# BenjSta/bernoulli-var-speech-codec

Hardware: AMD Instinct MI355X
Metric: audio-seconds coded per wall-second (encode+decode), 22.05 kHz @ 3 kbit/s (higher is better)
Workload: dtype f32; 1 GPU; BASELINE configs[1]: batch 64 x 5 s utterances per GPU, config_varBitRate @ 3000 bit/s (35 bits/frame), full encode -> BigVGAN decode; one batch at a time on one stream; frames_per_utterance=430, weights=seeded synthetic (checkpoints are LFS pointers), gather=none, streams=1

## Files before the change

bernoulli-var-speech-codec_amd/_abi.py:

```python
import ctypes
import os

import torch

_HERE = os.path.dirname(os.path.abspath(__file__))
LIB_PATH = os.environ.get("BVC_LIB") or os.path.join(_HERE, "csrc", "libbvcodec_hip.so")

c_float_p = ctypes.POINTER(ctypes.c_float)


class BvcConfig(ctypes.Structure):
    _fields_ = [
        ("num_mels", ctypes.c_int32), ("h_dim", ctypes.c_int32), ("z_dim", ctypes.c_int32),
        ("var_bit", ctypes.c_int32), ("n_fft", ctypes.c_int32), ("hop", ctypes.c_int32),
        ("pad_left", ctypes.c_int32), ("sample_rate", ctypes.c_int32),
        ("fmin", ctypes.c_float), ("fmax", ctypes.c_float),
        ("upsample_initial_channel", ctypes.c_int32), ("n_up", ctypes.c_int32),
        ("up_rates", ctypes.c_int32 * 8), ("up_kernels", ctypes.c_int32 * 8),
        ("n_resk", ctypes.c_int32), ("res_kernels", ctypes.c_int32 * 4),
        ("res_dilations", (ctypes.c_int32 * 3) * 4),
    ]


class BvcTensor(ctypes.Structure):
# ... 22 lines not shown
                                         _vp, _sz, _vp]),
    "bvc_bigvgan": (ctypes.c_int, [_vp, _vp, _i32, _i64, _i64, _f, _vp, _vp, _sz, _vp]),
    "bvc_vocoder_stream_create": (ctypes.c_int, [_vp, _i32, _i32, ctypes.POINTER(_vp)]),
    "bvc_vocoder_stream_destroy": (None, [_vp]),
    "bvc_vocoder_stream_reset": (ctypes.c_int, [_vp, _vp]),
    "bvc_vocoder_stream_push": (ctypes.c_int, [_vp, _vp, _i32, _f, _vp, _vp]),
    "bvc_stream_codec_create": (ctypes.c_int, [_vp, _i32, _i32, _f, _f, _f, ctypes.POINTER(_vp)]),
    "bvc_stream_codec_destroy": (None, [_vp]),
    "bvc_stream_codec_buffers": (ctypes.c_int, [_vp, ctypes.POINTER(_vp), ctypes.POINTER(_vp), ctypes.POINTER(_vp), ctypes.POINTER(_i32)]),
    "bvc_stream_codec_tick": (ctypes.c_int, [_vp, ctypes.POINTER(_i32), _vp]),
    "bvc_stream_codec_open": (ctypes.c_int, [_vp, _i32, _f, ctypes.POINTER(_i32)]),
    "bvc_stream_codec_close": (ctypes.c_int, [_vp, _i32]),
    "bvc_stream_codec_set_bits": (ctypes.c_int, [_vp, _i32, _f]),
    "bvc_stream_codec_slot_frames": (ctypes.c_int, [_vp, _i32, ctypes.POINTER(_i32), ctypes.POINTER(_i32), ctypes.POINTER(_i64)]),
    "bvc_encode": (ctypes.c_int, [_vp, _vp, _i32, _i64, _f, _f, _vp, _vp, _sz, _vp]),
    "bvc_decode": (ctypes.c_int, [_vp, _vp, _i32, _i64, _i64, _f, _vp, _vp, _sz, _vp]),
    "bvc_forward": (ctypes.c_int, [_vp, _vp, _i32, _i64, _f, _f, _i64, _f, _vp, _vp, _vp, _sz, _vp]),
    "bvc_encode_ragged": (ctypes.c_int, [_vp, _vp, _vp, _i32, _i64, _f, _vp, _f, _vp, _vp, _sz, _vp]),
    "bvc_decode_ragged": (ctypes.c_int, [_vp, _vp, _vp, _i32, _i64, _vp, _i64, _f, _vp, _vp, _sz, _vp]),
    "bvc_resample_poly": (ctypes.c_int, [_vp, _i32, _i64, _vp, _i32, _i32, _i32, _i64, _vp, _i64, _vp]),
    "bvc_peak_normalize": (ctypes.c_int, [_vp, _i32, _i64, _vp]),
    "bvc_pack_codes": (ctypes.c_int, [_vp, _i32, _i64, _i32, _i32, _vp, _vp]),
    "bvc_unpack_codes": (ctypes.c_int, [_vp, _i32, _i64, _i32, _i32, _vp, _vp]),
    "bvc_probe_begin": (ctypes.c_int, [_i32, _i32, _i32]),
    "bvc_probe_end": (ctypes.c_int, [ctypes.POINTER(ctypes.c_double), ctypes.POINTER(ctypes.c_double),
                                     ctypes.POINTER(_i32)]),
    "bvc_kprobe_enable": (ctypes.c_int, [_i32]),
    "bvc_kprobe_read": (ctypes.c_int, [_i32, _i32, ctypes.POINTER(ctypes.c_double), ctypes.POINTER(ctypes.c_double),
                                       ctypes.POINTER(_i32)]),
    "bvc_kprobe_read_span": (ctypes.c_int, [_i32, _i32, _i32, _i32, ctypes.POINTER(ctypes.c_double),
                                            ctypes.POINTER(ctypes.c_double), ctypes.POINTER(_i32)]),
    "bvc_test_linear": (ctypes.c_int, [_vp, _vp, _vp, _i32, _i32, _i32, _i32, _vp, _vp]),
    "bvc_test_linear_batched": (ctypes.c_int, [_vp, _vp, _vp, _i32, _i32, _i32, _i32, _vp, _vp]),
    "bvc_test_snakebeta": (ctypes.c_int, [_vp, _i64, _f, _f, _vp, _vp]),
    "bvc_test_vocoder_tap": (ctypes.c_int, [_vp, _vp, _i32, _i64, _i32, _vp, ctypes.POINTER(_i64), _vp, _sz, _vp]),
}

_lib = None


class BvcError(RuntimeError):
    pass


def load():
    global _lib
    if _lib is None:
        if not os.path.exists(LIB_PATH):
            raise BvcError(f"{LIB_PATH} is missing: build it with `python -m bvcodec.build` "
                           "(or __graft_entry__.build()); this package has no CPU fallback")
        lib = ctypes.CDLL(LIB_PATH)
        for name, (res, args) in SIGNATURES.items():
            fn = getattr(lib, name)
            fn.restype, fn.argtypes = res, args
        if lib.bvc_abi_version() != 3:
            raise BvcError("libbvcodec_hip.so ABI version mismatch")
        _lib = lib
    return _lib


def check(rc):
    if rc != 0:
        msg = load().bvc_last_error()
        raise BvcError(f"bvcodec error {rc}: {msg.decode() if msg else ''}")


# ... 10 lines not shown
```

bernoulli-var-speech-codec_amd/csrc/bvc_internal.h:

```cpp
#pragma once
#include <hip/hip_runtime.h>
#include <stdint.h>
#include <string>
#include <vector>

#include "../../include/bvcodec.h"

namespace bvc {

void set_error(const char *fmt, ...);

#define BVC_HIP_TRY(expr)                                                              \
    do {                                                                               \
        hipError_t e_ = (expr);                                                        \
        if (e_ != hipSuccess) {                                                        \
            bvc::set_error("%s failed: %s (%s:%d)", #expr, hipGetErrorString(e_), __FILE__, __LINE__); \
            return BVC_EHIP;                                                           \
        }                                                                              \
    } while (0)

enum ProbeKind { PK_NONE = 0, PK_LINEAR = 1, PK_GRU = 2, PK_CONV = 3, PK_BATCHED = 4, PK_STFT = 5, PK_POST = 6 };
struct ProbeScope {
    hipStream_t s; int slot;
    ProbeScope(int kind, hipStream_t stream);
// ... 48 lines not shown
};
enum CodeSample {
    CS_ENCODE = 0,
    CS_GREEDY = 1,
    CS_SAMPLE = 2
};

struct GemmParams {
    int     M, N;
    int     nb_total;
    int     gate_rows;
    GemmSeg seg[3];
    int     nseg;
    int     var_bit;
    int     sample;
    int     gate_il;
    const float *bias0;
    const float *bias1;
    DynPtr  y, y2, y3;
    DynPtr  aux;
    const float *part_i; const float *part_h; long long ldpart;
    const float *mean; const float *stdv;
    const CallDesc *desc;
    unsigned long long *probe;
    int     node;
    int     tstep;
    int     frames;
};

int launch_gemm_skinny(const GemmParams &p, int epi, hipStream_t s, int mtw = 1);
int skinny_kernels_init();
int launch_step_advance(CallDesc *d, int by, hipStream_t s);
int launch_set_desc(CallDesc *d, const CallDesc &v, hipStream_t s);

enum GemmOut { GO_NATURAL = 0, GO_FRAME_MAJOR_ROWS = 1, GO_PACKED_FRAMES = 2, GO_PACKED_FROM_UTT = 3 };
int launch_gemm_batched(const float *x, long long ldx, const float *w, long long ldw, const float *bias,
                        int M, int N, int K, int act, float *y, long long ldy, hipStream_t s,
                        int out_mode = GO_NATURAL, long long frames_T = 0, int mt16 = 0);
int launch_normalize_rows(const float *y, const float *mean, const float *stdv, long long rows, int n,
                          float *out, hipStream_t s);
int launch_fill(float *p, float v, long long n, hipStream_t s);
int launch_kld_frames(const float *prob, const float *prior, const float *bits, int B, long long T, int Z, float *kld,
                      hipStream_t s);
int launch_copy_rows(const float *src, long long lds, float *dst, long long ldd, int rows, int n, hipStream_t s);
int launch_repack_rows(const float *src, float *dst, long long ld_natural, int rows, int n, int dir, hipStream_t s);

constexpr unsigned FLOW_POISON = 0xFFFFDEADu;
constexpr int FLOW_STAMPS = 6;
enum FlowEpi { FE_ELU = 0, FE_CODE = 1, FE_MEL = 2, FE_GRU = 3, FE_ELU_KEEP = 4 };
enum FlowBuf { FB_H = 0, FB_E1, FB_E2, FB_ZC, FB_Q1, FB_Q2, FB_Q3, FB_D1, FB_D2, FB_D3, FB_DN, FB_G1, FB_G2, FB_G3, FB_COUNT };
struct FlowLin {
    const float *w;
    const float *bias;
    int wnb;
    int pad_;
};
struct FlowArgs {
    FlowLin enc0h, enc1, enc2, pz0, pz1, pz2, dec0h, dec0z, dec1, dec2, dec3, px0, px1, px2;
    const float *w_hh, *w_ihx, *w_ihz;
    const float *b_ih, *b_hh;
    int hb, zb, xb;
    float *flow; unsigned slot_bytes;
    int B, MT, NTG;
    long long T;
    const float *part0;
    const float *part_gru;
// ... 90 lines not shown
```

bernoulli-var-speech-codec_amd/csrc/bvcodec_abi.hip:

```cpp
#include <algorithm>
#include <atomic>
#include <cmath>
#include <cstdarg>
#include <cstdio>
#include <cstdlib>
#include <cstring>
#include <list>
#include <map>
#include <memory>
#include <mutex>

#include "bvc_internal.h"

namespace bvc {

static thread_local char g_err[512] = "";

void set_error(const char *fmt, ...) {
    va_list ap;
    va_start(ap, fmt);
    vsnprintf(g_err, sizeof(g_err), fmt, ap);
    va_end(ap);
}

// ... 2432 lines not shown
                }
                const unsigned long long b = h[(size_t)to * per + t * g_kprobe.nodes + k];
                if (!a || b <= a) continue;
                const double us = (double)(b - a) * 0.01;
                sum += us; if (us < mn) mn = us; ++n;
            }
    }
    if (mean_us) *mean_us = n ? sum / n : 0.0;
    if (min_us) *min_us = n ? mn : 0.0;
    if (n_samples) *n_samples = n;
    return BVC_OK;
}

int bvc_test_linear(const float *d_x, const float *d_w, const float *d_bias, int32_t M, int32_t N, int32_t K,
                    int32_t act, float *d_y, void *stream) {
    if (K % 16 || N % 16) { set_error("bvc_test_linear: N and K must be multiples of 16"); return BVC_EINVAL; }
    float *wp = nullptr;
    BVC_HIP_TRY(hipMalloc(reinterpret_cast<void **>(&wp), (size_t)N * K * sizeof(float)));
    hipStream_t s = (hipStream_t)stream;
    int rc = launch_repack_rows(d_w, wp, K, N, K, 0, s);
    Linear l; l.w = d_w; l.wp = wp; l.b = d_bias; l.in = K; l.out = N;
    if (!rc) rc = launch_gemm_skinny(lin_params(l, dp_static(d_x, K), M, dp_static(d_y, N)), act ? EPI_ELU : EPI_LINEAR, s);
    hipError_t e = hipStreamSynchronize(s);
    (void)hipFree(wp);
    if (!rc && e != hipSuccess) { set_error("bvc_test_linear: %s", hipGetErrorString(e)); rc = BVC_EHIP; }
    return rc;
}

int bvc_test_linear_batched(const float *d_x, const float *d_w, const float *d_bias, int32_t M, int32_t N, int32_t K,
                            int32_t act, float *d_y, void *stream) {
    return launch_gemm_batched(d_x, K, d_w, K, d_bias, M, N, K, act, d_y, N, (hipStream_t)stream);
}

int bvc_test_snakebeta(const float *d_x, int64_t n, float alpha, float beta, float *d_y, void *stream) {
    if (!d_x || !d_y || n <= 0) { set_error("bvc_test_snakebeta: bad arguments"); return BVC_EINVAL; }
    const float a = (float)std::exp((double)alpha);
    const float ib = 1.0f / ((float)std::exp((double)beta) + 0.000000001f);
    return launch_snakebeta_test(d_x, n, a, ib, d_y, (hipStream_t)stream);
}

int bvc_test_vocoder_tap(const bvc_model *m, const float *d_mel, int32_t B, int64_t T, int32_t which, float *d_out,
                         int64_t *out_numel_per_batch, void *d_ws, size_t ws_bytes, void *stream) {
    Workspace w;
    int rc = check_ws(m, B, T, d_ws, ws_bytes, &w);
    if (rc) return rc;
    if (which < 0 || which > 2 * m->cfg.n_up) { set_error("tap index out of range"); return BVC_EINVAL; }
    const float *tap = nullptr;
    int64_t len = 0;
    int ch = 0;
    hipStream_t s = (hipStream_t)stream;
    if ((rc = run_vocoder(m, w, d_mel, B, T, 1, 1.0f, nullptr, which, &tap, &len, &ch, s))) return rc;
    const long long n = (long long)B * len * ch;
    if (out_numel_per_batch) *out_numel_per_batch = len * ch;
    if (d_out) {
        hipLaunchKernelGGL(tap_copy_kernel, dim3(1024), dim3(256), 0, s, tap, d_out, n);
        BVC_HIP_TRY(hipGetLastError());
    }
    return BVC_OK;
}

}
```

bernoulli-var-speech-codec_amd/csrc/k_gemm.hip:

```cpp
#include <cstdlib>

#include <cstdint>
#include <type_traits>

#include "bvc_internal.h"

namespace bvc {

typedef float f32x4 __attribute__((ext_vector_type(4)));

__device__ __forceinline__ f32x4 mfma16(float a, float b, f32x4 c) {
    return __builtin_amdgcn_mfma_f32_16x16x4f32(a, b, c, 0, 0, 0);
}

__device__ __forceinline__ float elu1(float v) { return v > 0.0f ? v : expf(v) - 1.0f; }
__device__ __forceinline__ float sigmoid1(float v) { return 1.0f / (1.0f + expf(-v)); }

struct Resolved { float *p; long long ld; bool ok; int packed; };

__device__ __forceinline__ int sload_i32(const void *p) {
    int v;
    asm volatile("s_load_dword %0, %1, 0x0\n\ts_waitcnt lgkmcnt(0)" : "=s"(v) : "s"(p) : "memory");
    return v;
}
__device__ __forceinline__ long long sload_i64(const void *p) {
    long long v;
    asm volatile("s_load_dwordx2 %0, %1, 0x0\n\ts_waitcnt lgkmcnt(0)" : "=s"(v) : "s"(p) : "memory");
    return v;
}

template <bool MF = false>
__device__ __forceinline__ Resolved resolve(const DynPtr &d, const CallDesc *c, int mt16, int tstep) {
// ... 590 lines not shown
            if (row >= M) continue;
#pragma unroll
            for (int j = 0; j < 4; ++j) {
                const int col = n0 + j * 16 + g * 4;
                const f32x4 b4 = bias ? *reinterpret_cast<const f32x4 *>(bias + col) : (f32x4){0.f, 0.f, 0.f, 0.f};
                f32x4 v = acc[i][j] + b4;
                if (ACT == 1) {
#pragma unroll
                    for (int e = 0; e < 4; ++e) v[e] = elu1(v[e]);
                }
                *reinterpret_cast<f32x4 *>(y + out_index(row, col, N, ldy, frames_T, mt16, out_mode)) = v;
            }
        }
        return;
    }
#pragma unroll
    for (int j = 0; j < 4; ++j) {
        const int col = n0 + j * 16 + r;
        const float b = bias ? bias[col] : 0.0f;
#pragma unroll
        for (int i = 0; i < MI; ++i)
#pragma unroll
            for (int e = 0; e < 4; ++e) {
                const int row = m0 + i * 16 + g * 4 + e;
                if (row < M) {
                    float v = acc[i][j][e] + b;
                    if (ACT == 1) v = elu1(v);
                    y[out_index(row, col, N, ldy, frames_T, mt16, out_mode)] = v;
                }
            }
    }
}

int launch_gemm_batched(const float *x, long long ldx, const float *w, long long ldw, const float *bias,
                        int M, int N, int K, int act, float *y, long long ldy, hipStream_t s, int out_mode,
                        long long frames_T, int mt16) {
    if (M <= 0) return BVC_OK;
    if (K % 16 || ldx % 4 || ldw % 4) {
        set_error("gemm_batched: K=%d ldx=%lld ldw=%lld must be multiples of 16/4/4", K, ldx, ldw);
        return BVC_EINVAL;
    }
    if (out_mode != GO_NATURAL) {
        const bool utt_rows = out_mode == GO_FRAME_MAJOR_ROWS || out_mode == GO_PACKED_FROM_UTT;
        if (mt16 <= 0 || mt16 % 16 || N % 16 || (utt_rows && (frames_T <= 0 || M % frames_T || M / frames_T > mt16)) ||
            (out_mode == GO_PACKED_FRAMES && M % mt16)) {
            set_error("gemm_batched: inconsistent frame layout (M=%d T=%lld mt16=%d N=%d mode=%d)", M, frames_T, mt16, N, out_mode);
            return BVC_EINVAL;
        }
    }
    dim3 grid((N + 127) / 128, (M + 127) / 128);
    ProbeScope probe(PK_BATCHED, s);
    static const bool no_lds = getenv("BVC_NO_LDS_GEMM") != nullptr;
    if (!no_lds && K % 256 == 0 && N % 128 == 0) {
        const size_t lds = (size_t)2 * 2 * 128 * 36 * sizeof(float);
        static bool attr = false;
        if (!attr) {
            const void *ks[] = {(const void *)gemm_batched_lds_kernel<0, 128, false>, (const void *)gemm_batched_lds_kernel<1, 128, false>,
                                (const void *)gemm_batched_lds_kernel<0, 64, false>,  (const void *)gemm_batched_lds_kernel<1, 64, false>,
                                (const void *)gemm_batched_lds_kernel<0, 32, false>,  (const void *)gemm_batched_lds_kernel<1, 32, false>,
                                (const void *)gemm_batched_lds_kernel<0, 128, true>,  (const void *)gemm_batched_lds_kernel<1, 128, true>,
                                (const void *)gemm_batched_lds_kernel<0, 64, true>,   (const void *)gemm_batched_lds_kernel<1, 64, true>,
                                (const void *)gemm_batched_lds_kernel<0, 32, true>,   (const void *)gemm_batched_lds_kernel<1, 32, true>};
            for (const void *k : ks) BVC_HIP_TRY(hipFuncSetAttribute(k, hipFuncAttributeMaxDynamicSharedMemorySize, (int)lds));
            attr = true;
        }
        const bool rv = N % 4 == 0 && ldy % 4 == 0 && (reinterpret_cast<uintptr_t>(y) & 15) == 0 && (!bias || (reinterpret_cast<uintptr_t>(bias) & 15) == 0);
        auto launch = [&](auto act_c, auto bm_c, dim3 grid_, int m_off_) {
            constexpr int A_ = decltype(act_c)::value, BM_ = decltype(bm_c)::value;
            const size_t lds_ = (size_t)2 * (BM_ + 128) * 36 * sizeof(float);
            if (rv) hipLaunchKernelGGL((gemm_batched_lds_kernel<A_, BM_, true>), grid_, dim3(256), lds_, s, x, ldx, w, ldw, bias, M, N, K, y, ldy, frames_T, mt16, out_mode, m_off_);
            else    hipLaunchKernelGGL((gemm_batched_lds_kernel<A_, BM_, false>), grid_, dim3(256), lds_, s, x, ldx, w, ldw, bias, M, N, K, y, ldy, frames_T, mt16, out_mode, m_off_);
        };
        static const bool no_tail = getenv("BVC_NO_GEMM_TAIL") != nullptr;
        static const bool no_q = getenv("BVC_NO_GEMM_QUARTER") != nullptr;
        const int ncol = N / 128, rows_blk = (M + 127) / 128;
        const int slots = 512, per_round = slots / ncol > 0 ? slots / ncol : 1;
        int full_blk = rows_blk;
        if (!no_tail && rows_blk > per_round && rows_blk % per_round != 0 && (rows_blk % per_round) * 2 <= per_round)
            full_blk = (rows_blk / per_round) * per_round;
        if (full_blk > 0) {
            dim3 g1(ncol, full_blk);
            if (act == 1) launch(std::integral_constant<int, 1>(), std::integral_constant<int, 128>(), g1, 0);
            else          launch(std::integral_constant<int, 0>(), std::integral_constant<int, 128>(), g1, 0);
        }
        if (full_blk < rows_blk) {
            const int m_off = full_blk * 128;
            const int q_tiles = ncol * ((M - m_off + 31) / 32);
            if (!no_q && q_tiles <= 768) {
                dim3 g2(ncol, (M - m_off + 31) / 32);
                if (act == 1) launch(std::integral_constant<int, 1>(), std::integral_constant<int, 32>(), g2, m_off);
                else          launch(std::integral_constant<int, 0>(), std::integral_constant<int, 32>(), g2, m_off);
            } else {
                dim3 g2(ncol, (M - m_off + 63) / 64);
                if (act == 1) launch(std::integral_constant<int, 1>(), std::integral_constant<int, 64>(), g2, m_off);
                else          launch(std::integral_constant<int, 0>(), std::integral_constant<int, 64>(), g2, m_off);
            }
        }
        BVC_HIP_TRY(hipGetLastError());
        return BVC_OK;
    }
    const bool rowvec = out_mode == GO_NATURAL && N % 4 == 0 && ldy % 4 == 0 && (reinterpret_cast<uintptr_t>(y) & 15) == 0 &&
                        (!bias || (reinterpret_cast<uintptr_t>(bias) & 15) == 0);
    if (rowvec) {
        if (act == 1) hipLaunchKernelGGL((gemm_batched_kernel<1, true>), grid, dim3(256), 0, s, x, ldx, w, ldw, bias, M, N, K, y, ldy, frames_T, mt16, out_mode);
        else          hipLaunchKernelGGL((gemm_batched_kernel<0, true>), grid, dim3(256), 0, s, x, ldx, w, ldw, bias, M, N, K, y, ldy, frames_T, mt16, out_mode);
    } else if (act == 1)
        hipLaunchKernelGGL(gemm_batched_kernel<1>, grid, dim3(256), 0, s, x, ldx, w, ldw, bias, M, N, K, y, ldy, frames_T, mt16, out_mode);
    else
        hipLaunchKernelGGL(gemm_batched_kernel<0>, grid, dim3(256), 0, s, x, ldx, w, ldw, bias, M, N, K, y, ldy, frames_T, mt16, out_mode);
    BVC_HIP_TRY(hipGetLastError());
    return BVC_OK;
}

__global__ void normalize_rows_kernel(const float *__restrict__ y, const float *__restrict__ mean,
                                      const float *__restrict__ stdv, long long total, int n,
                                      float *__restrict__ out) {
    for (long long i = (long long)blockIdx.x * blockDim.x + threadIdx.x; i < total;
         i += (long long)gridDim.x * blockDim.x) {
        const int c = (int)(i % n);
        out[i] = (y[i] - mean[c]) / stdv[c];
    }
// ... 101 lines not shown
```

bernoulli-var-speech-codec_amd/csrc/k_vocoder.hip:

```cpp
#include <cstdlib>
#include <type_traits>

#include "bvc_internal.h"

namespace bvc {

typedef float f32x4 __attribute__((ext_vector_type(4)));

__device__ __forceinline__ void divide_if(bool div, f32x4 &v, float d) {
    if (div) {
        asm volatile("" ::: "memory");
#pragma unroll
        for (int e = 0; e < 4; ++e) v[e] = v[e] / d;
    }
}

__device__ __forceinline__ unsigned div_tpb(unsigned bid, unsigned tpb_magic) { return __umulhi(bid, tpb_magic); }
static inline unsigned tpb_magic_of(unsigned d) { return d <= 1u ? 0xFFFFFFFFu : (unsigned)(0x100000000ull / d) + 1u; }

__device__ __forceinline__ __amdgpu_buffer_rsrc_t rows_rsrc(const float *base, long long L, int C) {
    return __builtin_amdgcn_make_buffer_rsrc(const_cast<float *>(base), 0, (int)(L * C * 4), 0x00020000);
}
__device__ __forceinline__ f32x4 rows_load4(__amdgpu_buffer_rsrc_t rs, int row, int C, int c0) {
    return __builtin_bit_cast(f32x4, __builtin_amdgcn_raw_buffer_load_b128(rs, (row * C + c0) * 4, 0, 0));
// ... 902 lines not shown
        default: return -1;
    }
}
template <int MT>
static bool amp16_slots_all() {
    return amp16_slots<3, 1, MT, Amp16Occ<3, MT>::V>() > 0 && amp16_slots<3, 3, MT, Amp16Occ<3, MT>::V>() > 0 && amp16_slots<3, 5, MT, Amp16Occ<3, MT>::V>() > 0 &&
           amp16_slots<7, 1, MT, Amp16Occ<7, MT>::V>() > 0 && amp16_slots<7, 3, MT, Amp16Occ<7, MT>::V>() > 0 && amp16_slots<7, 5, MT, Amp16Occ<7, MT>::V>() > 0 &&
           amp16_slots<11, 1, (MT > 4 ? 4 : MT), Amp16Occ<11, MT>::V>() > 0 && amp16_slots<11, 3, (MT > 4 ? 4 : MT), Amp16Occ<11, MT>::V>() > 0 &&
           amp16_slots<11, 5, (MT > 4 ? 4 : MT), Amp16Occ<11, MT>::V>() > 0;
}

template <int C, int MT, int OCC, bool ALIAS, int CS = 1>
static int launch_amp_t(AmpArgs a, int B, hipStream_t s) {
    constexpr int TR = (4 / CS) * MT * 16;
    const int TT = TR - (a.ks - 1);
    a.tiles_per_batch = (int)((a.L - a.row_begin + TT - 1) / TT);
    if (a.tiles_per_batch <= 0) return BVC_OK;
    a.tpb_magic = tpb_magic_of((unsigned)a.tiles_per_batch);
    if ((unsigned long long)a.tiles_per_batch * a.tiles_per_batch * (unsigned long long)B >= 0x100000000ull) { set_error("vocoder: tile count beyond the reciprocal's range"); return BVC_EINVAL; }
    const size_t lds = (size_t)((TR + (a.ks - 1) * a.dil) + (ALIAS ? 0 : TR + (a.ks - 1))) * (C + 2) * sizeof(float);
    if (lds > 160 * 1024 || TT <= 0) { set_error("amp_pair tile needs %zu B of LDS", lds); return BVC_EINVAL; }
    ProbeScope probe(PK_CONV, s);
    const unsigned ntile = (unsigned)(a.tiles_per_batch * (long long)B);
    a.ntile = ntile;
    {
        static bool attr = false;
        if (!attr) { BVC_HIP_TRY(hipFuncSetAttribute(reinterpret_cast<const void *>(amp_pair_kernel<C, MT, OCC, ALIAS, CS>), hipFuncAttributeMaxDynamicSharedMemorySize, 160 * 1024)); attr = true; }
    }
    hipLaunchKernelGGL((amp_pair_kernel<C, MT, OCC, ALIAS, CS>), dim3((ntile + 7u) & ~7u), dim3(256), lds, s, a);
    BVC_HIP_TRY(hipGetLastError());
    return BVC_OK;
}

int launch_amp_pair(const ConvLayer &c1, const ConvLayer &c2, const float *x, long long L, float *out, int B, int epi,
                    const float *acc, float divisor, hipStream_t s, const ConvWindow *win, unsigned kernels) {
    if (B <= 0 || L <= 0) return BVC_OK;
    if (c1.cin != c1.cout || c2.cin != c1.cin || c2.ks != c1.ks || c2.dil != 1 || !c1.act_a || !c2.act_a) {
        set_error("amp_pair: unsupported layer pair");
        return BVC_EINVAL;
    }
    AmpArgs a;
    a.x = x; a.out = out; a.acc = acc; a.L = L;
    a.w1 = c1.wp; a.b1 = c1.bias; a.a1 = c1.act_a; a.ib1 = c1.act_ib;
    a.w2 = c2.wp; a.b2 = c2.bias; a.a2 = c2.act_a; a.ib2 = c2.act_ib;
    if (c1.cin >= 32) {
        if (!c1.wp4 || !c2.wp4) { set_error("amp_pair: layer pair without the 16-byte weight packing"); return BVC_EINVAL; }
        a.w1 = c1.wp4; a.w2 = c2.wp4;
    }
    a.divisor = divisor; a.epi = epi; a.ks = c1.ks; a.dil = c1.dil; a.tiles_per_batch = 0;
    a.bs = win ? win->in_bs : L * c1.cin;
    a.row_begin = win ? win->row_begin : 0;
    a.t_origin = win ? win->t_origin : 0;
    a.row_age = win ? win->row_age : nullptr;
    a.age_rate = win ? win->age_rate : 0;
    const long long new_rows = L - a.row_begin;
    if (win && c1.cin == 64 && new_rows <= 32 - (c1.ks - 1)) return launch_amp_t<64, 2, 2, true, 4>(a, B, s);
    if (win && c1.cin == 64 && new_rows <= 2 * (64 - (c1.ks - 1))) return launch_amp_t<64, 1, 2, true>(a, B, s);
    static const int s32 = getenv("BVC_AMP32S") ? atoi(getenv("BVC_AMP32S")) : 3;
    if (win && c1.cin == 32 && new_rows <= s32 * (64 - (c1.ks - 1))) return launch_amp_t<32, 1, 3, true>(a, B, s);
    if (c1.cin == 8 && c1.wp2 && c2.wp2 && (kernels & AMPK_C8)) {
        AmpArgs a8 = a;
        a8.w1 = c1.wp2; a8.w2 = c2.wp2;
        const int rc8 = (win && new_rows <= 128) ? launch_amp8<1, 4>(a8, B, s) : launch_amp8<2, 2>(a8, B, s);
        if (rc8 != -1) return rc8;
    }
    switch (c1.cin) {
        case 64: {
            static const bool rows = getenv("BVC_AMP64") && atoi(getenv("BVC_AMP64")) == 0;
            if (rows) return launch_amp_t<64, 2, 2, true>(a, B, s);
            return launch_amp_t<64, 8, 2, true, 4>(a, B, s);
        }
        case 32: return launch_amp_t<32, 4, 3, true>(a, B, s);
        case 16: {
            if ((kernels & AMPK_C16) && !win) {
                const int rc16 = launch_amp16<4>(a, B, s);
                if (rc16 != -1) return rc16;
            }
            return launch_amp_t<16, 2, 4, false>(a, B, s);
        }
        case 8:  return launch_amp_t<8, 4, 4, true>(a, B, s);
        default: set_error("amp_pair: unsupported channel count %d", c1.cin); return BVC_EINVAL;
    }
}

template <int CIN, int NTW, int MT, bool NSPLIT = false>
static int launch_one(const ConvArgs &a, int B, hipStream_t s) {
    constexpr int TT = (NSPLIT ? 1 : 4) * MT * 16;
    ConvArgs k = a;
    k.tiles_per_batch = (int)((a.Lout - a.row_begin + TT - 1) / TT);
    if (k.tiles_per_batch <= 0) return BVC_OK;
    const size_t lds = (size_t)(TT + (a.ks - 1) * a.dil) * (CIN + 2) * sizeof(float);
    if (lds > 160 * 1024) { set_error("conv tile needs %zu B of LDS", lds); return BVC_EINVAL; }
    constexpr int NPW = NTW * (NSPLIT ? 4 : 1);
    dim3 grid((unsigned)(k.tiles_per_batch * (long long)B), (unsigned)((a.ntiles + NPW - 1) / NPW));
    auto kern = conv_mfma_kernel<CIN, NTW, MT, NSPLIT>;
    ProbeScope probe(PK_CONV, s);
    hipLaunchKernelGGL(kern, grid, dim3(256), lds, s, k);
    BVC_HIP_TRY(hipGetLastError());
    return BVC_OK;
}

template <int CIN, int NTW, int MT, bool NSPLIT = false>
static int allow_big_lds() {
// ... 155 lines not shown
```

include/bvcodec.h:

```cpp
#ifndef BVCODEC_H
#define BVCODEC_H

#include <stddef.h>
#include <stdint.h>

#ifdef __cplusplus
extern "C" {
#endif

#define BVC_ABI_VERSION 3

enum {
    BVC_OK = 0,
    BVC_EINVAL = -1,
    BVC_ENOMEM = -2,
    BVC_EHIP = -3,
    BVC_EMISSING = -4,
    BVC_ENODEVICE = -5,
    BVC_ETIMEOUT = -6
};

typedef struct bvc_config {
    int32_t num_mels;
    int32_t h_dim;
// ... 78 lines not shown
int  bvc_stream_codec_open(bvc_stream_codec *st, int32_t slot, float bits_per_frame, int32_t *delay_samples);
int  bvc_stream_codec_close(bvc_stream_codec *st, int32_t slot);
int  bvc_stream_codec_set_bits(bvc_stream_codec *st, int32_t slot, float bits_per_frame);
int  bvc_stream_codec_slot_frames(bvc_stream_codec *st, int32_t slot, int32_t *first, int32_t *count, int64_t *stream_frame0);

int bvc_encode(const bvc_model *m, const float *d_wav, int32_t B, int64_t L, float scale,
               float bits_per_frame, float *d_codes, void *d_ws, size_t ws_bytes, void *stream);

int bvc_decode(const bvc_model *m, const float *d_codes, int32_t B, int64_t T, int64_t length,
               float out_scale_div, float *d_wav, void *d_ws, size_t ws_bytes, void *stream);

int bvc_encode_ragged(const bvc_model *m, const float *d_wav, const int64_t *d_lengths, int32_t B, int64_t L, float scale,
                      const float *d_bits, float bits_per_frame, float *d_codes, void *d_ws, size_t ws_bytes, void *stream);
int bvc_decode_ragged(const bvc_model *m, const float *d_codes, const int64_t *d_frames, int32_t B, int64_t T,
                      const int64_t *d_lengths, int64_t n_max, float out_scale_div, float *d_wav, void *d_ws, size_t ws_bytes,
                      void *stream);

int bvc_forward(const bvc_model *m, const float *d_wav, int32_t B, int64_t L, float scale, float bits_per_frame, int64_t length,
                float out_scale_div, float *d_codes, float *d_wav_out, void *d_ws, size_t ws_bytes, void *stream);

int bvc_resample_poly(const float *d_x, int32_t B, int64_t L_in, const double *d_h, int32_t ntaps, int32_t up,
                      int32_t down, int64_t n_pre_remove, float *d_y, int64_t n_out, void *stream);
int bvc_peak_normalize(float *d_x, int32_t B, int64_t L, void *stream);

int bvc_pack_codes(const float *d_codes, int32_t B, int64_t T, int32_t z_dim, int32_t nbits, uint8_t *d_bytes,
                   void *stream);
int bvc_unpack_codes(const uint8_t *d_bytes, int32_t B, int64_t T, int32_t z_dim, int32_t nbits, float *d_codes,
                     void *stream);

int bvc_test_linear(const float *d_x, const float *d_w, const float *d_bias, int32_t M, int32_t N,
                    int32_t K, int32_t act, float *d_y, void *stream);
int bvc_test_linear_batched(const float *d_x, const float *d_w, const float *d_bias, int32_t M,
                            int32_t N, int32_t K, int32_t act, float *d_y, void *stream);
int bvc_test_vocoder_tap(const bvc_model *m, const float *d_mel, int32_t B, int64_t T, int32_t which,
                         float *d_out, int64_t *out_numel_per_batch, void *d_ws, size_t ws_bytes,
                         void *stream);

int bvc_test_snakebeta(const float *d_x, int64_t n, float alpha, float beta, float *d_y, void *stream);

int bvc_probe_begin(int32_t kind, int32_t sample_every, int32_t max_samples);
int bvc_probe_end(double *mean_us, double *min_us, int32_t *n_samples);
int bvc_kprobe_enable(int32_t on);
int bvc_kprobe_read(int32_t node_lo, int32_t node_hi, double *mean_us, double *min_us, int32_t *n_samples);
int bvc_kprobe_read_span(int32_t from, int32_t to, int32_t node_lo, int32_t node_hi, double *mean_us, double *min_us,
                         int32_t *n_samples);

#ifdef __cplusplus
}
#endif
#endif
```

Measured before the change: 6974 audio-seconds/s.

## Choose GEMM and amp-pair tile heights from a wave-quantization cost model

Adds a tile-planning cost model that picks the row-tile height from a small set (144/128/112 for batched GEMM, 128/112/96/80 for the 64-channel amp pair) to minimise scheduling rounds over a fixed number of slots. A new column-oriented batched GEMM kernel with a fragment ring and variable tile height replaces the old 128-row path by default, and the amp-pair 64 kernel's per-block row count now follows the same plan. The aim is to cut partial last waves of tiles on the GPU. The cost is more kernel instantiations and a model that may not match real per-tile cost, plus trace and test hooks.

```diff
diff --git a/bernoulli-var-speech-codec_amd/_abi.py b/bernoulli-var-speech-codec_amd/_abi.py
--- a/bernoulli-var-speech-codec_amd/_abi.py
+++ b/bernoulli-var-speech-codec_amd/_abi.py
@@ -78,6 +78,7 @@
                                             ctypes.POINTER(ctypes.c_double), ctypes.POINTER(_i32)]),
     "bvc_test_linear": (ctypes.c_int, [_vp, _vp, _vp, _i32, _i32, _i32, _i32, _vp, _vp]),
     "bvc_test_linear_batched": (ctypes.c_int, [_vp, _vp, _vp, _i32, _i32, _i32, _i32, _vp, _vp]),
+    "bvc_test_tile_plan": (ctypes.c_int, [_i32, _i64, _i32, _i32, _i32, ctypes.POINTER(_i64)]),
     "bvc_test_snakebeta": (ctypes.c_int, [_vp, _i64, _f, _f, _vp, _vp]),
     "bvc_test_vocoder_tap": (ctypes.c_int, [_vp, _vp, _i32, _i64, _i32, _vp, ctypes.POINTER(_i64), _vp, _sz, _vp]),
 }
diff --git a/bernoulli-var-speech-codec_amd/csrc/bvc_internal.h b/bernoulli-var-speech-codec_amd/csrc/bvc_internal.h
--- a/bernoulli-var-speech-codec_amd/csrc/bvc_internal.h
+++ b/bernoulli-var-speech-codec_amd/csrc/bvc_internal.h
@@ -104,6 +104,29 @@
 int skinny_kernels_init();
 int launch_step_advance(CallDesc *d, int by, hipStream_t s);
 int launch_set_desc(CallDesc *d, const CallDesc &v, hipStream_t s);
+
+struct TilePlan { int height; long long tiles, rounds, cost; };
+inline TilePlan tile_plan(long long rows, long long column_blocks, const int *heights, const int *slots_for_height, int n,
+                          int fixed, int overlap = 0) {
+    TilePlan best = {0, 0, 0, 0};
+    if (rows <= 0 || column_blocks <= 0) return best;
+    for (int i = 0; i < n; ++i) {
+        const int h = heights[i], out_rows = h - overlap, slots = slots_for_height[i];
+        if (out_rows <= 0 || slots <= 0) continue;
+        const long long tiles = column_blocks * ((rows + out_rows - 1) / out_rows);
+        const long long rounds = (tiles + slots - 1) / slots;
+        const long long cost = rounds * (h + fixed);
+        if (best.height == 0 || cost < best.cost || (cost == best.cost && h > best.height)) best = {h, tiles, rounds, cost};
+    }
+    return best;
+}
+struct GemmCut { int height; int full_blocks; int tail_height; long long tiles, rounds, cost100; };
+GemmCut gemm_batched_cut(int M, int N, int force_height = 0, bool legacy = false);
+TilePlan amp_pair_cut(long long L, int B, int ks, int force_height = 0, bool legacy = false);
+bool tile_cut_legacy();
+void tile_trace(const char *what, long long rows, long long cols, int height, int tail_height, long long tiles, int slots, long long rounds);
+extern GemmCut g_last_gemm_cut;
+extern TilePlan g_last_amp_cut;
 
 enum GemmOut { GO_NATURAL = 0, GO_FRAME_MAJOR_ROWS = 1, GO_PACKED_FRAMES = 2, GO_PACKED_FROM_UTT = 3 };
 int launch_gemm_batched(const float *x, long long ldx, const float *w, long long ldw, const float *bias,
diff --git a/bernoulli-var-speech-codec_amd/csrc/bvcodec_abi.hip b/bernoulli-var-speech-codec_amd/csrc/bvcodec_abi.hip
--- a/bernoulli-var-speech-codec_amd/csrc/bvcodec_abi.hip
+++ b/bernoulli-var-speech-codec_amd/csrc/bvcodec_abi.hip
@@ -2488,6 +2488,21 @@
     return launch_gemm_batched(d_x, K, d_w, K, d_bias, M, N, K, act, d_y, N, (hipStream_t)stream);
 }
 
+int bvc_test_tile_plan(int32_t kind, int64_t rows, int32_t column_blocks, int32_t ks, int32_t mode, int64_t *out) {
+    if (!out || kind < 0 || kind > 1) { set_error("bvc_test_tile_plan: bad arguments"); return BVC_EINVAL; }
+    const bool last = mode == -1, legacy = mode == 1;
+    const int force = mode >= 16 ? mode : 0;
+    if (kind == 0) {
+        const GemmCut c = last ? g_last_gemm_cut : gemm_batched_cut((int)rows, column_blocks * 128, force, legacy);
+        out[0] = c.height; out[1] = c.full_blocks; out[2] = c.tail_height; out[3] = c.tiles; out[4] = c.rounds; out[5] = c.cost100;
+        return BVC_OK;
+    }
+    const TilePlan c = last ? g_last_amp_cut : amp_pair_cut(rows, column_blocks, ks, force, legacy);
+    out[0] = c.height; out[1] = c.height ? c.tiles / (column_blocks > 0 && !last ? column_blocks : 1) : 0; out[2] = 0;
+    out[3] = c.tiles; out[4] = c.rounds; out[5] = c.cost * 100;
+    return BVC_OK;
+}
+
 int bvc_test_snakebeta(const float *d_x, int64_t n, float alpha, float beta, float *d_y, void *stream) {
     if (!d_x || !d_y || n <= 0) { set_error("bvc_test_snakebeta: bad arguments"); return BVC_EINVAL; }
     const float a = (float)std::exp((double)alpha);
diff --git a/bernoulli-var-speech-codec_amd/csrc/k_gemm.hip b/bernoulli-var-speech-codec_amd/csrc/k_gemm.hip
--- a/bernoulli-var-speech-codec_amd/csrc/k_gemm.hip
+++ b/bernoulli-var-speech-codec_amd/csrc/k_gemm.hip
@@ -1,3 +1,4 @@
+#include <cstdio>
 #include <cstdlib>
 
 #include <cstdint>
@@ -654,6 +655,243 @@
     }
 }
 
+struct OutRow { long long base; int bb; };
+__device__ __forceinline__ OutRow out_row(int row, int N, long long ldy, long long T, int mt16, int mode) {
+    if (mode == GO_NATURAL) return {(long long)row * ldy, 0};
+    if (mode == GO_PACKED_FRAMES) {
+        const int tt = row / mt16;
+        return {(long long)tt * mt16 * N, row - tt * mt16};
+    }
+    const int Ti = (int)T;
+    const int bb = row / Ti;
+    const long long tt = row - bb * Ti;
+    if (mode == GO_FRAME_MAJOR_ROWS) return {(tt * mt16 + bb) * ldy, 0};
+    return {tt * (long long)mt16 * N, bb};
+}
+__device__ __forceinline__ long long out_at(const OutRow &o, int col, int N, int mode) {
+    return mode <= GO_FRAME_MAJOR_ROWS ? o.base + col : o.base + packed_off(o.bb, col, N);
+}
+
+template <int ACT, int BM, bool ROWVEC = false>
+__global__ __launch_bounds__(256, 2) void gemm_batched_cols_kernel(const float *__restrict__ x, long long ldx,
+                                                                   const float *__restrict__ w, long long ldw,
+                                                                   const float *__restrict__ bias, int M, int N,
+                                                                   int K, float *__restrict__ y, long long ldy,
+                                                                   long long frames_T, int mt16, int out_mode, int m_off) {
+    constexpr int BK = 32, LDT = BK + 4;
+    static_assert(BM % 16 == 0 && BM >= 48 && BM <= 144, "tile heights: 2 x 2 x (BM + 128) x 36 floats of LDS per CU");
+    constexpr int MI = BM / 16;
+    constexpr int PA = (BM + 31) / 32;
+    constexpr int NS = 2 * MI;
+    constexpr int RING = NS % 4 == 0 ? 4 : NS % 6 == 0 ? 6 : NS % 5 == 0 ? 5 : 7;
+    constexpr int D = RING - 1;
+    static_assert(NS % RING == 0 && MI >= D && NS - D >= MI, "fragment ring");
+    extern __shared__ __attribute__((aligned(16))) float smem[];
+    const int tid = threadIdx.x, lane = tid & 63;
+    const int wave = __builtin_amdgcn_readfirstlane(tid >> 6);
+    const int r = lane & 15, g = lane >> 4;
+    const int mblk = m_off + blockIdx.y * BM, nblk = blockIdx.x * 128;
+    const int wn = wave * 32;
+
+    const int srow = tid >> 3, spc = (tid & 7) * 4;
+    const int xrows = M - mblk < PA * 32 ? M - mblk : PA * 32;
+    const __amdgpu_buffer_rsrc_t xrs = __builtin_amdgcn_make_buffer_rsrc(const_cast<float *>(x + (long long)mblk * ldx), 0, (int)(xrows * ldx * 4), 0x00020000);
+    const __amdgpu_buffer_rsrc_t wrs = __builtin_amdgcn_make_buffer_rsrc(const_cast<float *>(w + (long long)nblk * ldw), 0, (int)(128 * ldw * 4), 0x00020000);
+    int xvo[PA];
+#pragma unroll
+    for (int p = 0; p < PA; ++p) xvo[p] = ((srow + 32 * p < xrows ? srow + 32 * p : xrows - 1) * (int)ldx + spc) * 4;
+    const int wvo = (srow * (int)ldw + spc) * 4;
+    f32x4 acc[MI][2], tot[MI][2];
+#pragma unroll
+    for (int i = 0; i < MI; ++i)
+#pragma unroll
+        for (int j = 0; j < 2; ++j) { acc[i][j] = (f32x4){0.f, 0.f, 0.f, 0.f}; tot[i][j] = (f32x4){0.f, 0.f, 0.f, 0.f}; }
+
+    constexpr int STAGE = (BM + 128) * LDT;
+    const int nk = K / BK;
+    const int cst = nk >> 3;
+    f32x4 ga[PA], gb[4];
+    auto gload = [&](int kt) {
+        const int ko = (kt < nk ? kt : nk - 1) * BK;
+#pragma unroll
+        for (int p = 0; p < PA; ++p) ga[p] = __builtin_bit_cast(f32x4, __builtin_amdgcn_raw_buffer_load_b128(xrs, xvo[p], ko * 4, 0));
+#pragma unroll
+        for (int p = 0; p < 4; ++p) gb[p] = __builtin_bit_cast(f32x4, __builtin_amdgcn_raw_buffer_load_b128(wrs, wvo, (32 * p * (int)ldw + ko) * 4, 0));
+    };
+    auto park = [&](float *A) {
+        float *B = A + BM * LDT;
+#pragma unroll
+        for (int p = 0; p < PA; ++p)
+            if (32 * (p + 1) <= BM || srow + 32 * p < BM) *reinterpret_cast<f32x4 *>(A + (srow + 32 * p) * LDT + spc) = ga[p];
+#pragma unroll
+        for (int p = 0; p < 4; ++p) *reinterpret_cast<f32x4 *>(B + (srow + 32 * p) * LDT + spc) = gb[p];
+    };
+    auto lds_barrier = [&]() {
+        asm volatile("s_waitcnt lgkmcnt(0)" ::: "memory");
+        __builtin_amdgcn_s_barrier();
+        asm volatile("" ::: "memory");
+    };
+    const int fo = r * LDT + g * 4;
+    auto lda = [&](const float *buf, int s) {
+        return *reinterpret_cast<const f32x4 *>(buf + fo + (s % MI) * 16 * LDT + (s / MI) * 16);
+    };
+    auto ldb = [&](const float *buf, int h, int j) {
+        return *reinterpret_cast<const f32x4 *>(buf + fo + (BM + wn + j * 16) * LDT + h * 16);
+    };
+    f32x4 ring[RING], bq[2][2];
+    gload(0);
+    park(smem);
+    gload(1);
+    lds_barrier();
+#pragma unroll
+    for (int s = 0; s < D; ++s) ring[s] = lda(smem, s);
+#pragma unroll
+    for (int j = 0; j < 2; ++j) bq[0][j] = ldb(smem, 0, j);
+
+    auto stage = [&](int kt) {
+        const float *cur = smem + (kt & 1) * STAGE;
+        float *nxt = smem + ((kt + 1) & 1) * STAGE;
+#pragma unroll
+        for (int s = 0; s < NS; ++s) {
+            const int h = s / MI, i = s % MI;
+            if (s == NS - D) {
+                park(nxt);
+                __builtin_amdgcn_sched_barrier(0);
+                gload(kt + 2);
+                lds_barrier();
+#pragma unroll
+                for (int j = 0; j < 2; ++j) bq[0][j] = ldb(nxt, 0, j);
+            }
+            if (s == MI - D) {
+#pragma unroll
+                for (int j = 0; j < 2; ++j) bq[1][j] = ldb(cur, 1, j);
+            }
+            ring[(s + D) % RING] = s + D < NS ? lda(cur, s + D) : lda(nxt, s + D - NS);
+            __builtin_amdgcn_sched_barrier(0);
+#pragma unroll
+            for (int e = 0; e < 4; ++e)
+#pragma unroll
+                for (int j = 0; j < 2; ++j) {
+                    acc[i][j] = ROWVEC ? mfma16(bq[h][j][e], ring[s % RING][e], acc[i][j]) : mfma16(ring[s % RING][e], bq[h][j][e], acc[i][j]);
+                }
+            __builtin_amdgcn_sched_barrier(0);
+        }
+    };
+    int in_chunk = 0;
+    for (int kt = 0; kt < nk; ++kt) {
+        stage(kt);
+        if (++in_chunk == cst) {
+            in_chunk = 0;
+#pragma unroll
+            for (int i = 0; i < MI; ++i)
+#pragma unroll
+                for (int j = 0; j < 2; ++j) { tot[i][j] += acc[i][j]; acc[i][j] = (f32x4){0.f, 0.f, 0.f, 0.f}; }
+        }
+    }
+
+    const int n0 = nblk + wn;
+    if (ROWVEC) {
+        f32x4 b4[2];
+#pragma unroll
+        for (int j = 0; j < 2; ++j) b4[j] = bias ? *reinterpret_cast<const f32x4 *>(bias + n0 + j * 16 + g * 4) : (f32x4){0.f, 0.f, 0.f, 0.f};
+#pragma unroll
+        for (int i = 0; i < MI; ++i) {
+            const int row = mblk + i * 16 + r;
+            if (row >= M) continue;
+            const OutRow o = out_row(row, N, ldy, frames_T, mt16, out_mode);
+#pragma unroll
+            for (int j = 0; j < 2; ++j) {
+                f32x4 v = tot[i][j] + b4[j];
+                if (ACT == 1) {
+#pragma unroll
+                    for (int e = 0; e < 4; ++e) v[e] = elu1(v[e]);
+                }
+                *reinterpret_cast<f32x4 *>(y + out_at(o, n0 + j * 16 + g * 4, N, out_mode)) = v;
+            }
+        }
+        return;
+    }
+#pragma unroll
+    for (int i = 0; i < MI; ++i)
+#pragma unroll
+        for (int e = 0; e < 4; ++e) {
+            const int row = mblk + i * 16 + g * 4 + e;
+            if (row >= M) continue;
+            const OutRow o = out_row(row, N, ldy, frames_T, mt16, out_mode);
+#pragma unroll
+            for (int j = 0; j < 2; ++j) {
+                const int col = n0 + j * 16 + r;
+                float v = tot[i][j][e] + (bias ? bias[col] : 0.0f);
+                if (ACT == 1) v = elu1(v);
+                y[out_at(o, col, N, out_mode)] = v;
+            }
+        }
+}
+
+bool tile_cut_legacy() {
+    const char *v = getenv("BVC_TILE_CUT");
+    return v != nullptr && v[0] == 'l';
+}
+void tile_trace(const char *what, long long rows, long long cols, int height, int tail_height, long long tiles, int slots, long long rounds) {
+    static const bool on = getenv("BVC_TILE_TRACE") != nullptr;
+    if (!on) return;
+    static long long seen[64][4];
+    static int nseen = 0;
+    const long long key[4] = {(long long)what[0] * 256 + what[1], rows, cols, height * 1000 + tail_height};
+    for (int i = 0; i < nseen; ++i)
+        if (seen[i][0] == key[0] && seen[i][1] == key[1] && seen[i][2] == key[2] && seen[i][3] == key[3]) return;
+    if (nseen < 64) { for (int q = 0; q < 4; ++q) seen[nseen][q] = key[q]; ++nseen; }
+    fprintf(stderr, "tile_trace %s rows=%lld cols=%lld height=%d tail_height=%d tiles=%lld slots=%d rounds=%lld (%.2f needed)\n", what, rows, cols,
+            height, tail_height, tiles, slots, rounds, (double)tiles / slots);
+}
+
+GemmCut g_last_gemm_cut = {0, 0, 0, 0, 0, 0};
+static constexpr int GEMM_FIXED_ROWS = 1;
+static constexpr int GEMM_SLOTS = 512;
+GemmCut gemm_batched_cut(int M, int N, int force_height, bool legacy) {
+    GemmCut c = {0, 0, 0, 0, 0, 0};
+    if (M <= 0 || N < 128) return c;
+    const int ncol = N / 128, rows_blk = (M + 127) / 128;
+    static const bool no_tail = getenv("BVC_NO_GEMM_TAIL") != nullptr;
+    static const bool no_q = getenv("BVC_NO_GEMM_QUARTER") != nullptr;
+    const int per_round = GEMM_SLOTS / ncol > 0 ? GEMM_SLOTS / ncol : 1;
+    int full_blk = rows_blk;
+    if (!no_tail && rows_blk > per_round && rows_blk % per_round != 0 && (rows_blk % per_round) * 2 <= per_round)
+        full_blk = (rows_blk / per_round) * per_round;
+    GemmCut two = {128, full_blk, 0, 0, 0, 0};
+    two.tiles = (long long)ncol * full_blk;
+    two.rounds = (two.tiles + GEMM_SLOTS - 1) / GEMM_SLOTS;
+    two.cost100 = two.rounds * 100 * (128 + GEMM_FIXED_ROWS);
+    if (full_blk < rows_blk) {
+        const int m_off = full_blk * 128;
+        const long long q_tiles = (long long)ncol * ((M - m_off + 31) / 32), h_tiles = (long long)ncol * ((M - m_off + 63) / 64);
+        const bool quarter = !no_q && q_tiles <= 768;
+        two.tail_height = quarter ? 32 : 64;
+        const long long t_tiles = quarter ? q_tiles : h_tiles, t_slots = quarter ? 768 : GEMM_SLOTS;
+        const long long t_rounds = (t_tiles + t_slots - 1) / t_slots;
+        two.tiles += t_tiles; two.rounds += t_rounds;
+        two.cost100 += t_rounds * (quarter ? 46 : 55) * (128 + GEMM_FIXED_ROWS);
+    }
+    if (legacy && force_height == 0) return two;
+    static const int heights[3] = {144, 128, 112}, slots[3] = {GEMM_SLOTS, GEMM_SLOTS, GEMM_SLOTS};
+    TilePlan p;
+    if (force_height) {
+        int one = 0;
+        for (int h : heights) if (h == force_height) one = h;
+        if (!one) return c;
+        p = tile_plan(M, ncol, &one, slots, 1, GEMM_FIXED_ROWS);
+    } else {
+        p = tile_plan(M, ncol, heights, slots, 3, GEMM_FIXED_ROWS);
+    }
+    if (!force_height && two.tail_height != 0 && two.cost100 < p.cost * 100) return two;
+    c.height = p.height; c.full_blocks = (M + p.height - 1) / p.height; c.tail_height = 0;
+    c.tiles = p.tiles; c.rounds = p.rounds; c.cost100 = p.cost * 100;
+    return c;
+}
+
+#define BVC_COLS_KERNELS(BM) (const void *)gemm_batched_cols_kernel<0, BM, false>, (const void *)gemm_batched_cols_kernel<1, BM, false>, \
+                             (const void *)gemm_batched_cols_kernel<0, BM, true>,  (const void *)gemm_batched_cols_kernel<1, BM, true>
+
 int launch_gemm_batched(const float *x, long long ldx, const float *w, long long ldw, const float *bias,
                         int M, int N, int K, int act, float *y, long long ldy, hipStream_t s, int out_mode,
                         long long frames_T, int mt16) {
@@ -693,22 +931,47 @@
             if (rv) hipLaunchKernelGGL((gemm_batched_lds_kernel<A_, BM_, true>), grid_, dim3(256), lds_, s, x, ldx, w, ldw, bias, M, N, K, y, ldy, frames_T, mt16, out_mode, m_off_);
             else    hipLaunchKernelGGL((gemm_batched_lds_kernel<A_, BM_, false>), grid_, dim3(256), lds_, s, x, ldx, w, ldw, bias, M, N, K, y, ldy, frames_T, mt16, out_mode, m_off_);
         };
-        static const bool no_tail = getenv("BVC_NO_GEMM_TAIL") != nullptr;
-        static const bool no_q = getenv("BVC_NO_GEMM_QUARTER") != nullptr;
-        const int ncol = N / 128, rows_blk = (M + 127) / 128;
-        const int slots = 512, per_round = slots / ncol > 0 ? slots / ncol : 1;
-        int full_blk = rows_blk;
-        if (!no_tail && rows_blk > per_round && rows_blk % per_round != 0 && (rows_blk % per_round) * 2 <= per_round)
-            full_blk = (rows_blk / per_round) * per_round;
-        if (full_blk > 0) {
+        const char *force = getenv("BVC_GEMM_BM");
+        const bool legacy = tile_cut_legacy();
+        const GemmCut cut = gemm_batched_cut(M, N, force ? atoi(force) : 0, legacy);
+        if (force && cut.height != atoi(force)) { set_error("gemm_batched: BVC_GEMM_BM=%s is not a compiled tile height", force); return BVC_EINVAL; }
+        g_last_gemm_cut = cut;
+        tile_trace("gemm_batched", M, N, cut.height, cut.tail_height, cut.tiles, 512, cut.rounds);
+        const int ncol = N / 128;
+        if (!legacy) {
+            static bool attr2 = false;
+            if (!attr2) {
+                const void *ks[] = {BVC_COLS_KERNELS(144), BVC_COLS_KERNELS(128), BVC_COLS_KERNELS(112)};
+                for (const void *k : ks) BVC_HIP_TRY(hipFuncSetAttribute(k, hipFuncAttributeMaxDynamicSharedMemorySize, 2 * (144 + 128) * 36 * (int)sizeof(float)));
+                attr2 = true;
+            }
+            auto launch_cols = [&](auto bm_c) {
+                constexpr int BM_ = decltype(bm_c)::value;
+                const dim3 grid_(ncol, cut.full_blocks);
+                const size_t lds_ = (size_t)2 * (BM_ + 128) * 36 * sizeof(float);
+                auto go = [&](auto kern) { hipLaunchKernelGGL(kern, grid_, dim3(256), lds_, s, x, ldx, w, ldw, bias, M, N, K, y, ldy, frames_T, mt16, out_mode, 0); };
+                if (act == 1) { if (rv) go(gemm_batched_cols_kernel<1, BM_, true>); else go(gemm_batched_cols_kernel<1, BM_, false>); }
+                else          { if (rv) go(gemm_batched_cols_kernel<0, BM_, true>); else go(gemm_batched_cols_kernel<0, BM_, false>); }
+            };
+            switch (cut.height) {
+                case 144: launch_cols(std::integral_constant<int, 144>()); break;
+                case 128: launch_cols(std::integral_constant<int, 128>()); break;
+                default:  launch_cols(std::integral_constant<int, 112>()); break;
+            }
+            if (cut.tail_height == 0) {
+                BVC_HIP_TRY(hipGetLastError());
+                return BVC_OK;
+            }
+        }
+        const int rows_blk = (M + 127) / 128, full_blk = cut.full_blocks;
+        if (full_blk > 0 && legacy) {
             dim3 g1(ncol, full_blk);
             if (act == 1) launch(std::integral_constant<int, 1>(), std::integral_constant<int, 128>(), g1, 0);
             else          launch(std::integral_constant<int, 0>(), std::integral_constant<int, 128>(), g1, 0);
         }
         if (full_blk < rows_blk) {
             const int m_off = full_blk * 128;
-            const int q_tiles = ncol * ((M - m_off + 31) / 32);
-            if (!no_q && q_tiles <= 768) {
+            if (cut.tail_height == 32) {
                 dim3 g2(ncol, (M - m_off + 31) / 32);
                 if (act == 1) launch(std::integral_constant<int, 1>(), std::integral_constant<int, 32>(), g2, m_off);
                 else          launch(std::integral_constant<int, 0>(), std::integral_constant<int, 32>(), g2, m_off);
diff --git a/bernoulli-var-speech-codec_amd/csrc/k_vocoder.hip b/bernoulli-var-speech-codec_amd/csrc/k_vocoder.hip
--- a/bernoulli-var-speech-codec_amd/csrc/k_vocoder.hip
+++ b/bernoulli-var-speech-codec_amd/csrc/k_vocoder.hip
@@ -958,6 +958,17 @@
     return BVC_OK;
 }
 
+TilePlan g_last_amp_cut = {0, 0, 0, 0};
+static constexpr int AMP64_FIXED_ROWS = 1;
+TilePlan amp_pair_cut(long long L, int B, int ks, int force_height, bool legacy) {
+    static const int heights[4] = {128, 112, 96, 80}, slots[4] = {512, 512, 512, 512};
+    if (!force_height && !legacy) return tile_plan(L, B, heights, slots, 4, AMP64_FIXED_ROWS, ks - 1);
+    int one = force_height ? 0 : heights[0];
+    for (int h : heights) if (h == force_height) one = h;
+    if (!one) return {0, 0, 0, 0};
+    return tile_plan(L, B, &one, slots, 1, AMP64_FIXED_ROWS, ks - 1);
+}
+
 int launch_amp_pair(const ConvLayer &c1, const ConvLayer &c2, const float *x, long long L, float *out, int B, int epi,
                     const float *acc, float divisor, hipStream_t s, const ConvWindow *win, unsigned kernels) {
     if (B <= 0 || L <= 0) return BVC_OK;
@@ -994,7 +1005,21 @@
         case 64: {
             static const bool rows = getenv("BVC_AMP64") && atoi(getenv("BVC_AMP64")) == 0;
             if (rows) return launch_amp_t<64, 2, 2, true>(a, B, s);
-            return launch_amp_t<64, 8, 2, true, 4>(a, B, s);
+            int tr = 128;
+            if (!win) {
+                const char *force = getenv("BVC_AMP64_TR");
+                const TilePlan cut = amp_pair_cut(new_rows, B, c1.ks, force ? atoi(force) : 0, tile_cut_legacy());
+                if (cut.height == 0) { set_error("amp_pair: BVC_AMP64_TR=%s is not a compiled tile height", force ? force : ""); return BVC_EINVAL; }
+                g_last_amp_cut = cut;
+                tile_trace("amp_pair64", new_rows, (long long)B * 100 + c1.ks, cut.height, 0, cut.tiles, 512, cut.rounds);
+                tr = cut.height;
+            }
+            switch (tr) {
+                case 80:  return launch_amp_t<64, 5, 2, true, 4>(a, B, s);
+                case 96:  return launch_amp_t<64, 6, 2, true, 4>(a, B, s);
+                case 112: return launch_amp_t<64, 7, 2, true, 4>(a, B, s);
+                default:  return launch_amp_t<64, 8, 2, true, 4>(a, B, s);
+            }
         }
         case 32: return launch_amp_t<32, 4, 3, true>(a, B, s);
         case 16: {
diff --git a/include/bvcodec.h b/include/bvcodec.h
--- a/include/bvcodec.h
+++ b/include/bvcodec.h
@@ -134,6 +134,7 @@
                     int32_t K, int32_t act, float *d_y, void *stream);
 int bvc_test_linear_batched(const float *d_x, const float *d_w, const float *d_bias, int32_t M,
                             int32_t N, int32_t K, int32_t act, float *d_y, void *stream);
+int bvc_test_tile_plan(int32_t kind, int64_t rows, int32_t column_blocks, int32_t ks, int32_t mode, int64_t *out);
 int bvc_test_vocoder_tap(const bvc_model *m, const float *d_mel, int32_t B, int64_t T, int32_t which,
                          float *d_out, int64_t *out_numel_per_batch, void *d_ws, size_t ws_bytes,
                          void *stream);
```

Measured after the change: 7092 audio-seconds/s (median of 6 runs). 1.02x the previous value.
